# ykevinc/pocket-tts

Measured on AMD Instinct MI355X. Metric: audio-sec/wall-sec (RTF) per GPU at batch=32 + p50 first-chunk latency, higher is better.
Workload: dtype f32; 1 GPU; b6369a24 batch=32 concurrent 10 s utterances per GPU (125 frames, voice prompt 125 frames, 40 text tokens), lsd_decode_steps=1 (BASELINE configs[2]); global_batch=32, utterance_frames=125, jobs=37, prompt_frames=125, parallelism=replicas x1

## Files before the change

pocket-tts_amd/csrc/capi.cpp:

```cpp
#include <cstdlib>
#include <cstring>
#include <string>

#include "engine.h"
#include "flac_join.h"
#include "pocket_tts.h"
#include "pocket_tts_probe.h"
#include "test_hooks.h"

struct ptts_engine {
  ptts::Engine* impl = nullptr;
};

namespace {
thread_local std::string g_err;

template <class F>
int guard(F&& f) {
  try {
    f();
    g_err.clear();
    return PTTS_OK;
  } catch (const ptts::Error& e) {
    g_err = e.what();
// ... 158 lines not shown
}

int ptts_resample(ptts_engine* e, const float* x, int n_samples, int sr_from, int sr_to, float* y) {
  return guard([&] { eng(e).resample_host(x, n_samples, sr_from, sr_to, y); });
}

int ptts_resample_len_ex(int n_samples, int sr_from, int sr_to, int resampler) {
  if (resampler == PTTS_RESAMPLE_POLY) return ptts_resample_len(n_samples, sr_from, sr_to);
  if (resampler != PTTS_RESAMPLE_RUBATO_SEPTIC || n_samples <= 0 || sr_from <= 0 || sr_to <= 0) return 0;
  if (sr_from == sr_to) return n_samples;
  const long n = ptts::septic_schedule(n_samples, sr_from, sr_to, nullptr, nullptr);
  return n < (1L << 30) ? (int)n : 0;
}

int ptts_resample_ex(ptts_engine* e, const float* x, int n_samples, int sr_from, int sr_to, int resampler, float* y) {
  return guard([&] { eng(e).resample_host(x, n_samples, sr_from, sr_to, y, resampler); });
}

int ptts_voice_from_audio_ex(ptts_engine* e, const float* samples, int n_samples, int sample_rate, int chunk_frames,
                             int resampler, ptts_voice** out) {
  return guard([&] {
    if (!out) throw ptts::Error(PTTS_ERR_INVALID, "null out");
    *out = eng(e).voice_from_audio(samples, n_samples, sample_rate, chunk_frames, resampler);
  });
}

int ptts_test_gemm(ptts_engine* e, int layout, int m, int n, int k, int splits, int tail_slices, const float* x,
                   const float* w, float* y) {
  return guard([&] { eng(e).test_gemm(layout, m, n, k, splits, tail_slices, x, w, y); });
}

int ptts_test_attention(ptts_engine* e, int kind, int m, int nh, int cap, int window, int n_slots, int splits,
                        const float* qkv, float* kv, const float* pre, const int* pre_len, int slot0, int rps, int p0,
                        const int* pos, const int* tab, const int* ptab, int mpad, float* q, float* o) {
  return guard([&] {
    eng(e).test_attention(kind, m, nh, cap, window, n_slots, splits, qkv, kv, pre, pre_len, slot0, rps, p0, pos, tab,
                          ptab, mpad, q, o);
  });
}

int ptts_test_align(ptts_engine* e, int m, int nh, int cap, int splits, const float* qkv, const float* kv,
                    const float* pre, const int* pre_len, const int* pos, const int* tab, unsigned head_mask,
                    float* out) {
  return guard([&] { eng(e).test_align(m, nh, cap, splits, qkv, kv, pre, pre_len, pos, tab, head_mask, out); });
}

int ptts_test_row_reduce(ptts_engine* e, int m, int n, int splits, int act, int ln, float eps, int front,
                         const float* p, const float* bias, const float* gate, const float* r, const float* ln_w,
                         const float* ln_b, const float* mscale, const float* mshift, float* y, float* h,
                         float* hfrag) {
  return guard([&] {
    eng(e).test_row_reduce(m, n, splits, act, ln, eps, front, p, bias, gate, r, ln_w, ln_b, mscale, mshift, y, h, hfrag);
  });
}

int ptts_voice_job_start(ptts_engine* e, const void* samples, int n_samples, int sample_format, int sample_rate,
                         int chunk_frames, int resampler, ptts_voice** out) {
  return guard([&] {
    if (!out) throw ptts::Error(PTTS_ERR_INVALID, "null out");
    *out = nullptr;
    *out = eng(e).voice_job_audio(samples, n_samples, sample_format, sample_rate, chunk_frames, resampler);
  });
}

int ptts_voice_job_start_prompt(ptts_engine* e, const float* prompt, int n_frames, ptts_voice** out) {
  return guard([&] {
    if (!out) throw ptts::Error(PTTS_ERR_INVALID, "null out");
    *out = nullptr;
    *out = eng(e).voice_job_prompt(prompt, n_frames);
  });
}

int ptts_voice_ready(const ptts_voice* v, int wait, int* ready) {
  return guard([&] {
    if (!ready) throw ptts::Error(PTTS_ERR_INVALID, "null argument");
    *ready = 1;
    if (!v || !v->ev) return;
    if (wait) {
      PTTS_HIP(hipEventSynchronize(v->ev));
      return;
    }
    const hipError_t q = hipEventQuery(v->ev);
    if (q == hipErrorNotReady) *ready = 0;
    else PTTS_HIP(q);
  });
}

int ptts_voice_jobs_reserve(ptts_engine* e, int max_frames) {
  return guard([&] { eng(e).voice_jobs_reserve(max_frames); });
}

int ptts_voice_len(const ptts_voice* v) { return v ? v->F : 0; }

int ptts_voice_conditioning(const ptts_voice* v, float* out, int max_rows) {
  return guard([&] {
    if (!v || !out) throw ptts::Error(PTTS_ERR_INVALID, "null argument");
    if (v->cond.empty() && !v->h_cond) throw ptts::Error(PTTS_ERR_STATE, "voice was not built from PCM");
    const int rows = std::min(max_rows, v->F);
    if (v->h_cond) {
      PTTS_HIP(hipEventSynchronize(v->ev));
      memcpy(out, v->h_cond, sizeof(float) * rows * ptts::D);
      return;
    }
    memcpy(out, v->cond.data(), sizeof(float) * rows * ptts::D);
  });
}
// ... 311 lines not shown
```

pocket-tts_amd/csrc/engine.cpp:

```cpp
#include "engine.h"

#include <hip/hip_ext.h>

#include <algorithm>
#include <array>
#include <cstdlib>
#include <cmath>
#include <cstring>
#include <mutex>

namespace ptts {

namespace {
std::mutex& voice_mu() {
  static std::mutex m;
  return m;
}

int pick_splits(int M, int N, int K) {
  const int tiles = ((N + 31) / 32) * ((M + 31) / 32);
  const int chunks = K / 32;
  int s = std::max(1, 768 / std::max(1, tiles));
  s = std::min(s, std::max(1, chunks / 4));
  return std::min(s, 16);
// ... 557 lines not shown
      use.push_back(&q);
      bytes += ((size_t)q.N * q.K + 255) / 256 * 256;
    }
  }
  if (use.empty()) return;
  void* codes = nullptr;
  PTTS_HIP(hipMalloc(&codes, bytes));
  allocs_.push_back(codes);
  int* bad = (int*)dalloc(1);
  size_t off = 0;
  for (const Layout::Q8* q : use) {
    int8_t* c = (int8_t*)codes + off;
    quant_codes(W(q->w), W(q->s), q->N, q->K, c, bad, stream_);
    q8map_[W(q->w)] = {c, W(q->s)};
    off += ((size_t)q->N * q->K + 255) / 256 * 256;
  }
  PTTS_HIP(hipGetLastError());
  int nbad = 0;
  PTTS_HIP(hipMemcpyAsync(&nbad, bad, sizeof(int), hipMemcpyDeviceToHost, stream_));
  PTTS_HIP(hipStreamSynchronize(stream_));
  if (nbad) {
    q8map_.clear();
    throw Error(PTTS_ERR_INVALID, "quantized weights are not on their int8 grid (" + std::to_string(nbad) +
                                      " elements): blob not packed by the quantizer");
  }
}

void Engine::derive_fp8() {
  std::vector<const Layout::Q8*> use;
  size_t bytes = 0, nsc = 0;
  for (const Layout::Q8& q : L_.q8)
    if ((long)q.N * q.K >= (2L << 20)) {
      use.push_back(&q);
      bytes += ((size_t)q.N * q.K + 255) / 256 * 256;
      nsc += (size_t)q.N;
    }
  void* codes = nullptr;
  PTTS_HIP(hipMalloc(&codes, std::max<size_t>(bytes, 1)));
  allocs_.push_back(codes);
  float* scales = dalloc(nsc);
  size_t off = 0, so = 0;
  for (const Layout::Q8* q : use) {
    uint8_t* c = (uint8_t*)codes + off;
    fp8_codes(W(q->w), q->N, q->K, c, scales + so, stream_);
    f8map_[W(q->w)] = {c, scales + so};
    off += ((size_t)q->N * q->K + 255) / 256 * 256;
    so += (size_t)q->N;
  }
  PTTS_HIP(hipGetLastError());
  PTTS_HIP(hipStreamSynchronize(stream_));
}

void Engine::linear_split(std::vector<Op>& ops, const std::string& name, const float* X, long ldx, int M,
                          const float* Wt, int N, int K, int* S_out, const FlowBufs& fb) {
  PTTS_REQUIRE(K % 32 == 0, "GEMM K must be a multiple of 32");
  int S = pick_splits(M, N, K);
  int layout = TILE_KSPLIT_4W, tail = 0;
  if (M <= 64 && N >= 3072) {
    layout = TILE_GLDS_32x128;
    S = std::max(1, std::min(8, K / 64));
  } else if (M >= 256) {
    layout = N >= 4096 && K <= 1024 ? TILE_ILV_128x64 : TILE_ILV_128x64_2CU;
    tail = N >= 4096 && K <= 1024 ? 2 : 4;
    S = 1;
  } else if (M <= 64 && K >= 4096) {
    S = 8;
  } else if (M <= 64 && N <= 512 && K == 512) {
    layout = TILE_KSPLIT_8W;
    S = 8;
  }
  auto gv = gvmap_.find(Wt);
  if (gv != gvmap_.end() && M <= 64 && (gemv_mask_ & gv->second.bit)) {
    const GemvShape g = gv->second.g;
    const float* P = gv->second.packed;
    const uint32_t* q8 = gv->second.q8;
    const float* sc = gv->second.scale;
    const int Sg = K / g.ks();
    PTTS_REQUIRE((size_t)Sg * M * N <= fb.pcap, "split-K partial buffer too small");
    float* part = fb.partial;
    const bool f8 = fp8_ && q8;
    ops.push_back({name, [=](hipStream_t s) { gemv_splitk(X, ldx, M, N, K, P, g, part, s, q8, sc, f8); }, 2.0 * M * N * K,
                   (q8 ? 1.0 * N * K + 4.0 * N : 4.0 * N * K) + 4.0 * ((double)M * K + (double)Sg * M * N)});
    *S_out = Sg;
    return;
  }
  auto f8 = f8map_.find(Wt);
  const bool wf8 = f8 != f8map_.end() && M <= 64;
  if (wf8) {
    layout = TILE_KSPLIT_4W;
    const int tiles = ((N + 63) / 64) * ((M + 31) / 32), nch = K / 32;
    S = 1;
    while (S < 16 && tiles * S < 256 && nch / (2 * S) >= 4) S *= 2;
    while ((nch + S - 1) / S > FP8_KSLICE_MAX / 32) ++S;
  }
  auto q8 = q8map_.find(Wt);
  const bool w8 = q8 != q8map_.end() && M <= 64 && (long)N * K >= (2L << 20);
  if (w8) {
    layout = TILE_KSPLIT_4W;
    const int tiles = ((N + 63) / 64) * ((M + 31) / 32);
    S = 1;
    while (S < 16 && tiles * S < 256 && (K / 32) / (2 * S) >= 4) S *= 2;
  }
  if (!w8 && !wf8) tile_override(name, layout, S);
  while (S > 1 && (size_t)S * M * N > fb.pcap) --S;
  PTTS_REQUIRE((size_t)S * M * N <= fb.pcap, "split-K partial buffer too small");
  GemmArgs a = dense_gemm(layout, M, N, K, X, ldx, Wt);
  if (w8) {
    a.Wq = q8->second.first;
    a.wscale = q8->second.second;
  }
  if (wf8) {
    PTTS_REQUIRE((K / 32 + S - 1) / S <= FP8_KSLICE_MAX / 32, "fp8 GEMM K slice too long");
    a.Wf8 = f8->second.first;
    a.wscale = f8->second.second;
  }
  a.S = S;
  a.partial = fb.partial;
  if (tail > 0 && S == 1 && !w8 && !wf8) {
    a.tail_S = tail;
    a.tail_slab = fb.tslab;
    a.tail_cap = fb.tail_cap;
    a.tickets = fb.tickets;
    a.tickets_cap = TICKETS;
  }
  a.w_nt = M <= 64 && layout != TILE_KSPLIT_4W;
  a.front = 1;
  ops.push_back({name, [a, S](hipStream_t s) { gemm(a, S, s); }, 2.0 * M * N * K,
                 (w8 || wf8 ? (double)N * K + 4.0 * N : 4.0 * N * K) + 4.0 * ((double)M * K + (double)S * M * N)});
  *S_out = S;
}

static Op rr_op(const std::string& name, const RowReduceArgs& a) {
  const double mn = (double)a.M * a.N;
  double f = mn * (a.S + 1 + (a.act ? 8 : 0) + (a.ln ? 8 : 0));
  double b = mn * a.S + (a.bias ? a.N : 0) + (a.gate ? (a.ldg ? mn : a.N) : 0) + (a.R ? mn : 0) + (a.Y ? mn : 0) +
             (a.Y2 ? mn : 0) + (a.euler ? 2.0 * a.M * 32 : 0);
  if (a.ln) b += mn + (a.ln_w ? 2.0 * a.N : 0) + (a.mshift ? 2.0 * mn : 0);
  if (a.fhm) b += mn * 2.0 / 3.0;
  if (a.fill) b += 4.0 * a.fill_n4;
  if (a.x0_hx) {
    b += (double)a.x0_B * (32 + 512) + 32.0 * 512;
    f += 2.0 * a.x0_B * 32 * 512;
  }
  return Op{name, [a](hipStream_t s) { row_reduce(a, s); }, f, 4.0 * b};
}

void Engine::push_rr(std::vector<Op>& ops, const std::string& name, const RowReduceArgs& r) {
  RowReduceArgs a = r;
  a.front = 1;
  ops.push_back(rr_op(name, a));
}

void Engine::dense_op(std::vector<Op>& ops, const std::string& name, const float* X, int M, const float* Wt, int N,
                      int K, const float* bias, int act, const float* rscale, const float* R, float* Y, int layout) {
  int ks = 1;
  tile_override(name, layout, ks);
  PTTS_REQUIRE(K % tile_of(layout).bk == 0, "GEMM K must be a multiple of the tile's BK");
  GemmArgs a = dense_gemm(layout, M, N, K, X, K, Wt);
  a.S = 1;
  a.bias = bias;
  a.act = act;
  a.rscale = rscale;
  a.R = R;
  a.ldr = N;
  a.Y = Y;
  a.ldy = N;
  attach_split(a);
  ops.push_back({name, [a](hipStream_t s) { gemm(a, 1, s); }, 2.0 * M * N * K,
                 4.0 * ((double)N * K + (double)M * K + (double)M * N * (R ? 2 : 1))});
}

void Engine::conv_op(std::vector<Op>& ops, const std::string& name, const float* X, int B, int T_in, int cin,
                     const float* H, int P, int stride, int elu, const float* Wt, int cout, int ktaps, int phases,
                     const float* bias, const float* R, float* Y, int T_out, int tstride, int layout, int elu_out,
                     float* Y2, int ksplit, float* slabs, size_t slab_cap) {
  tile_override(name, layout, ksplit);
  const TileInfo& tile = tile_of(layout);
  PTTS_REQUIRE(cin % tile.bk == 0, "conv cin must be a multiple of the tile's BK");
  PTTS_REQUIRE(ksplit == 1 || (phases == 1 && tile.lds_dma()), "K-split convs need a single-phase LDS-DMA tile");
  GemmArgs a{};
  a.mode = 1;
  a.layout = layout;
  a.Tq = T_in / stride;
  a.M = B * a.Tq;
  a.N = cout;
  a.K = ktaps * cin;
  a.Nw = (cout + 31) / 32 * 32;
  a.X = X;
  a.ldx = cin;
  a.H = H;
  a.P = P;
  a.T_in = T_in;
  a.stride_in = stride;
  a.cin = cin;
  a.elu_in = elu;
  a.W = Wt;
  a.w_phase_stride = (long)cout * ktaps * cin;
  a.S = 1;
  a.bias = bias;
  a.R = R;
  a.ldr = cout;
  a.Y = Y;
  a.ldy = cout;
  a.T_out = T_out;
  a.out_tstride = tstride;
  a.elu_out = elu_out;
  a.Y2 = Y2;
  const int nph = phases;
  attach_split(a);
  if (ksplit > 1) {
    PTTS_REQUIRE((size_t)ksplit * a.M * a.N <= slab_cap, "back split-K slab buffer too small");
    a.S = ksplit;
    a.partial = slabs;
    phases = ksplit;
  }
  ops.push_back({name, [a, phases](hipStream_t s) { gemm(a, phases, s); }, 2.0 * a.M * a.N * a.K * nph,
                 4.0 * ((double)nph * a.N * a.K + (double)B * T_in * cin +
                        (double)B * T_out * cout * ((R ? 2 : 1) + (Y2 ? 1 : 0)))});
}

void Engine::flow_layers(std::vector<Op>& ops, int M, RowMap map, bool step, bool out_norm, const std::string& tag,
                         const FlowBufs& fb, float* align_out) {
  PTTS_REQUIRE(!step || &fb == &fbm_, "step passes run on the engine's own buffers");
  for (int l = 0; l < NL; ++l) {
    const Layout::TL& t = L_.fl[l];
    const std::string p = tag + ".l" + std::to_string(l);
    KvStore kv = fb.kv;
    kv.base += (long)l * fb.kv_layer;
    if (kv.pre) kv.layer = l;
    int S = 1;
    linear_split(ops, p + ".qkv_gemm", fb.h, D, M, W(t.in_proj), 3 * D, D, &S, fb);
    if (step) {
      const float* P = fb.partial;
      float* O = fb.o;
      const float* rope = rope_;
      const double L = plan_ctx_ > 0 ? plan_ctx_ : max_ctx_ / 2.0;
      const double kvu = plan_kvu_ > 0 ? plan_kvu_ : M * L;
      ops.push_back({p + ".attention", [=](hipStream_t s) { attention_step_qkv(P, S, M, NH, map, kv, rope, O, s); },
                     (double)M * 4096.0 * L,
                     8192.0 * kvu + (double)M * (4.0 * (S * 3.0 * D + 2.0 * D + D) + 64.0 * 4 * 2)});
      if (align_out && l == align_layer_) {
        AlignArgs a{};
        a.P = P;
        a.S = S;
        a.M = M;
        a.nh = NH;
        a.pos = map.pos_arr;
        a.kv = kv;
        a.rope = rope;
        a.tab = align_tab_;
        a.head_mask = align_mask_;
        a.out = align_out;
        double rows = 0, keys = 0;
        for (int b = 0; b < M; ++b)
          if (slot_align_[b]) rows += 1, keys += slot_align_[b];
        const double h = __builtin_popcount(align_mask_);
        ops.push_back({p + ".align", [=](hipStream_t s) { align_step(a, s); }, h * keys * (128.0 + 8.0),
                       h * (256.0 * keys + rows * 4.0 * (S * 64.0 + 64.0)) + rows * 4.0 * ALIGN_ROW +
                           (M - rows) * 4.0 + M * 12.0});
      }
    } else {
      {
        const float* P = fb.partial;
        float* Q = fb.q;
        ops.push_back({p + ".qkv_rope", [=](hipStream_t s) { qkv_rope_append(P, S, nullptr, M, NH, map, kv, Q, s); }});
      }
      const float* Q = fb.q;
      float* O = fb.o;
      RowMap am = map;
      int Ma = M;
      if (map.ptab) {
        am.tab = map.ptab;
        Ma = map.mpad;
      }
      ops.push_back({p + ".attention", [=](hipStream_t s) { attention(Q, Ma, NH, am, kv, 0, O, s); }});
    }
    auto rr = [&](const std::string& name, int S2, int N, int act, bool resid, float* Y, const float* lnw,
                  const float* lnb, bool ln, float* Hout, float* Hfrag = nullptr, float* fill = nullptr,
                  long fill_n4 = 0) {
      RowReduceArgs a{};
      a.Hfrag = Hfrag;
      a.fill = fill;
      a.fill_n4 = fill_n4;
// ... 2 lines not shown
      a.M = M;
      a.N = N;
      a.act = act;
      if (resid) {
        a.R = fb.x;
        a.ldr = D;
      }
      a.Y = Y;
      a.ldy = N;
      a.ln = ln ? 1 : 0;
      a.ln_w = lnw;
      a.ln_b = lnb;
      a.eps = 1e-5f;
      a.Hout = Hout;
      a.ldh = N;
      push_rr(ops, name, a);
    };
    linear_split(ops, p + ".out_gemm", fb.o, D, M, W(t.out_proj), D, D, &S, fb);
    auto fk = step && gemv_fk_supported(M, FF, D) ? fkmap_.find(W(t.l1)) : fkmap_.end();
    const bool use_fk = fk != fkmap_.end() && hfrag_;
    rr(p + ".out_reduce_ln2", S, D, ACT_NONE, true, fb.x, W(t.n2w), W(t.n2b), true, fb.h, use_fk ? hfrag_ : nullptr);
    auto ffn = use_fk && ffn_hand_ ? ffnmap_.find(W(t.l2)) : ffnmap_.end();
    if (ffn != ffnmap_.end()) {
      static_assert(NL % 2 == 0, "the fused FFN's hand-off sets alternate by layer");
      const float *A = hfrag_, *P1 = fk->second, *P2 = ffn->second;
      float *hand = ffn_hand_, *Pp = fb.partial;
      int* err = herr_;
      const int set = l & 1;
      const int groups = ffn_groups_;
      auto f8 = ffn8map_.find(W(t.l2));
      const uint32_t *Q1 = nullptr, *Q2 = nullptr;
      const float *s1 = nullptr, *s2 = nullptr;
      if (f8 != ffn8map_.end()) {
        Q1 = f8->second.first.first;
        s1 = f8->second.first.second;
        Q2 = f8->second.second.first;
        s2 = f8->second.second.second;
      }
      const bool e4m3 = fp8_ && Q1;
      Op op{p + ".ffn", [=](hipStream_t s) { ffn_fused(A, M, P1, P2, groups, hand, set, Pp, err, s, Q1, s1, Q2, s2, e4m3); },
            2.0 * M * FF * D * 2,
            (Q1 ? 2.0 * FF * D + 8.0 * (FF + D) : 8.0 * FF * D) + 4.0 * ((double)M * D + (double)groups * M * D)};
      op.prep = [hand](hipStream_t s) { PTTS_HIP(hipMemsetD32Async(hand, 0xFFFFFFFFu, 2 * FFN_HAND_FLOATS, s)); };
      ops.push_back(op);
      S = groups;
    } else {
      if (use_fk) {
        const float* Pk = fk->second;
        const float* A = hfrag_;
        float* U = fb.u;
        ops.push_back({p + ".ff1_gemm", [=](hipStream_t s) { gemv_fk(A, M, FF, Pk, nullptr, ACT_GELU, U, FF, s); },
                       2.0 * M * FF * D, 4.0 * ((double)FF * D + (double)M * D + (double)M * FF)});
      } else {
        linear_split(ops, p + ".ff1_gemm", fb.h, D, M, W(t.l1), FF, D, &S, fb);
        rr(p + ".ff1_reduce_gelu", S, FF, ACT_GELU, false, fb.u, nullptr, nullptr, false, nullptr);
      }
      linear_split(ops, p + ".ff2_gemm", fb.u, FF, M, W(t.l2), D, FF, &S, fb);
    }
    if (l + 1 < NL)
      rr(p + ".ff2_reduce_ln1", S, D, ACT_NONE, true, fb.x, W(L_.fl[l + 1].n1w), W(L_.fl[l + 1].n1b), true, fb.h);
    else {
      const bool pre = step && out_norm && use_head_prelude(M);
      const long n4 = (long)lsd_ * ((M + 15) / 16) * HP_REGION_FLOATS / 4;
      rr(p + ".ff2_reduce_outnorm", S, D, ACT_NONE, true, fb.x, W(L_.out_norm_w), W(L_.out_norm_b), out_norm, fb.h,
         pre ? hfrag_ : nullptr, pre ? hp_hand_ : nullptr, pre ? n4 : 0);
    }
  }
}

void Engine::prefill_rows(std::vector<Op>& ops, int slot, int T, int p0, const FlowBufs& fb) {
  {
    float *x = fb.x, *h = fb.h;
    const float* w = W(L_.fl[0].n1w);
    const float* b = W(L_.fl[0].n1b);
    ops.push_back({"prefill.ln1", [=](hipStream_t s) { layernorm(x, D, h, D, T, D, w, b, 1e-5f, s); }});
  }
  RowMap map{slot, T, p0, nullptr};
  flow_layers(ops, T, map, false, false, "prefill", fb);
}

bool Engine::use_head_chain(int B) const {
  if (!flow_head_fits(B)) return false;
  if (flow_head_grid(B) > head_resident_) return false;
  return head_uniform_stride();
}

bool Engine::use_head_prelude(int B) const {
  return hp_w_ && head_prelude_supported(B, 1) && gemv_fk_supported(B, NCOND_PAD, D) && use_head_chain(B);
}

bool Engine::head_uniform_stride() const {
  const long s = (long)(L_.rb_w0[1] - L_.rb_w0[0]);
  for (int i = 1; i < FDEPTH; ++i)
    if ((long)(L_.rb_lnw[i] - L_.rb_lnw[i - 1]) != s || (long)(L_.rb_lnb[i] - L_.rb_lnb[i - 1]) != s ||
        (long)(L_.rb_w0[i] - L_.rb_w0[i - 1]) != s || (long)(L_.rb_b0[i] - L_.rb_b0[i - 1]) != s ||
        (long)(L_.rb_w2[i] - L_.rb_w2[i - 1]) != s || (long)(L_.rb_b2[i] - L_.rb_b2[i - 1]) != s)
      return false;
  return true;
}

void Engine::build_front(std::vector<Op>& ops, int B, int hb, int lsd_run) {
  PTTS_REQUIRE(lsd_run >= 1 && lsd_run <= lsd_, "lsd_run outside [1, cap]");
  int S = 1;
  const FlowBufs& fb = fbm_;
  flow_layers(ops, B, RowMap{0, 1, 0, fpos_}, true, true, "flow", fb, align_ ? align_block(hb) : nullptr);
  if (use_head_prelude(B)) {
    const int RG = (B + 15) / 16;
    const size_t r0 = (size_t)(RG * 16) * FD;
// ... 1116 lines not shown
      void* p = dalloc(bytes);
      PTTS_HIP(hipMemcpyAsync(p, src, bytes, hipMemcpyHostToDevice, stream_));
      return p;
    };
    const float* dqkv = (const float*)up(qkv, sizeof(float) * n_qkv);
    float* dkv = (float*)up(kvh, sizeof(float) * n_kv);
    float* dq = (float*)dalloc(sizeof(float) * Mq * d);
    float* dout = (float*)dalloc(sizeof(float) * M * d);
    PTTS_HIP(hipMemsetAsync(dq, 0, sizeof(float) * Mq * d, stream_));
    PTTS_HIP(hipMemsetAsync(dout, 0, sizeof(float) * M * d, stream_));
    RowMap map{slot0, rps, p0, nullptr};
    if (tab) {
      map = RowMap{0, 1, 0, nullptr, (const int*)up(tab, sizeof(int) * M)};
      if (ptab) {
        map.ptab = (const int*)up(ptab, sizeof(int) * mpad);
        map.mpad = mpad;
        map.qrow = (const int*)up(qrow.data(), sizeof(int) * M);
        map.orow = (const int*)up(orow.data(), sizeof(int) * mpad);
      }
    } else if (pos) {
      map.pos_arr = (const int*)up(pos, sizeof(int) * n_slots);
    }
    KvStore kv{dkv, (long)2 * nh * cap * 64, cap};
    if (pre) {
      const float* dpre = (const float*)up(pre, sizeof(float) * pre_floats);
      for (int sl = 0; sl < n_slots; ++sl) prep[sl] = dpre + pre_off[sl];
      kv.pre = (const float* const*)up(prep.data(), sizeof(float*) * n_slots);
      kv.pre_len = (const int*)up(pre_len, sizeof(int) * n_slots);
      kv.layer = 0;
    }
    if (kind == 0) {
      qkv_rope_append(S > 0 ? dqkv : nullptr, S, S > 0 ? nullptr : dqkv, M, nh, map, kv, dq, stream_);
      RowMap am = map;
      if (map.ptab) am.tab = map.ptab;
      attention(dq, Mq, nh, am, kv, window, dout, stream_);
    } else if (kind == 1) {
      attention16_qkv(dqkv, M, nh, map, kv, window, dout, stream_);
    } else {
      float* drope = (float*)dalloc(sizeof(float) * cap * 64);
      rope_table(drope, cap, stream_);
      attention_step_qkv(dqkv, S, M, nh, map, kv, drope, dout, stream_);
    }
    PTTS_HIP(hipGetLastError());
    PTTS_HIP(hipMemcpyAsync(kvh, dkv, sizeof(float) * n_kv, hipMemcpyDeviceToHost, stream_));
    if (kind == 0) PTTS_HIP(hipMemcpyAsync(Qh, dq, sizeof(float) * Mq * d, hipMemcpyDeviceToHost, stream_));
    PTTS_HIP(hipMemcpyAsync(Oh, dout, sizeof(float) * M * d, hipMemcpyDeviceToHost, stream_));
    PTTS_HIP(hipStreamSynchronize(stream_));
  } catch (...) {
    (void)hipStreamSynchronize(stream_);
    release();
    throw;
  }
  release();
}

void Engine::test_row_reduce(int M, int N, int S, int act, int ln, float eps, int front, const float* P,
                             const float* bias, const float* gate, const float* R, const float* ln_w,
                             const float* ln_b, const float* mscale, const float* mshift, float* Y, float* H,
                             float* Hfrag) {
  PTTS_REQUIRE(ready_, "engine weights not finalized");
  PTTS_REQUIRE(P && Y && M >= 1 && M <= 4096 && N >= 4 && N <= 8192 && N % 4 == 0 && S >= 1 && S <= 16,
               "test_row_reduce: bad shape");
  PTTS_REQUIRE(act == ACT_NONE || act == ACT_GELU, "test_row_reduce: act is none or GELU");
  PTTS_REQUIRE(!ln || (N <= 1024 && H), "test_row_reduce: LayerNorm rows are at most 1024 wide");
  PTTS_REQUIRE((ln_w == nullptr) == (ln_b == nullptr) && (mscale == nullptr) == (mshift == nullptr),
               "test_row_reduce: ln_w with ln_b, mscale with mshift");
  PTTS_REQUIRE(ln || (!ln_w && !mshift && !Hfrag), "test_row_reduce: affine, modulate and hfrag need ln");
  PTTS_REQUIRE(!Hfrag || (N == FK_K && M <= 32), "test_row_reduce: hfrag needs n == 1024 and m <= 32");
  sync();
  std::vector<void*> allocs;
  auto release = [&]() {
    for (void* p : allocs) (void)hipFree(p);
  };
  try {
    auto dalloc = [&](size_t floats) {
      void* p = nullptr;
      PTTS_HIP(hipMalloc(&p, sizeof(float) * std::max<size_t>(floats, 4)));
      allocs.push_back(p);
      return (float*)p;
    };
    auto up = [&](const float* src, size_t floats) -> float* {
      if (!src) return nullptr;
      float* p = dalloc(floats);
      PTTS_HIP(hipMemcpyAsync(p, src, sizeof(float) * floats, hipMemcpyHostToDevice, stream_));
      return p;
    };
    const size_t mn = (size_t)M * N;
    RowReduceArgs a{};
    a.P = up(P, (size_t)S * mn);
    a.S = S, a.M = M, a.N = N;
    a.bias = up(bias, N);
    a.act = act;
    a.gate = up(gate, mn), a.ldg = N;
    a.R = up(R, mn), a.ldr = N;
    a.Y = dalloc(mn), a.ldy = N;
    a.ln = ln ? 1 : 0;
    a.ln_w = up(ln_w, N), a.ln_b = up(ln_b, N);
    a.eps = eps;
    a.mscale = up(mscale, mn), a.mshift = up(mshift, mn), a.ldm = N;
    a.front = front ? 1 : 0;
    if (ln) a.Hout = dalloc(mn), a.ldh = N;
    if (Hfrag) {
      a.Hfrag = dalloc(FK_A_FLOATS);
      PTTS_HIP(hipMemsetAsync(a.Hfrag, 0, sizeof(float) * FK_A_FLOATS, stream_));
    }
    row_reduce(a, stream_);
// ... 1807 lines not shown
```

pocket-tts_amd/csrc/engine.h:

```cpp
#pragma once
#include <functional>
#include <map>
#include <string>
#include <vector>

#include "common.h"
#include "kernels.h"
#include "weights.h"

struct ptts_voice {
  int F = 0;
  float* kv = nullptr;
  std::vector<float> cond;
  const void* owner = nullptr;
  mutable int refs = 0;
  mutable bool dead = false;
  hipEvent_t ev = nullptr;
  float* h_cond = nullptr;
  mutable bool ordered = false;
};

namespace ptts {

struct VoicePlan;
// ... 36 lines not shown
  void slots_open(int n, const int* slots, const ptts_voice* const* voices, const int32_t* ids, const int* n_ids,
                  const ptts_gen_params* params, const ptts_slot_opts* opts);
  int lsd_cap() const { return lsd_; }
  int lsd_last_run() const { return lsd_last_run_; }
  void slot_close(int slot);
  void slots_cancel(int n, const int* slots);
  void set_latent(int slot, const float* lat);
  void decode_latents(int slot, const float* lat, int n, float* pcm, float* quant, float* up, float* tr);

  void step_async(int B);
  void flush_async(int B);
  void sync();
  void fetch(int B, float* pcm, uint8_t* valid, uint8_t* last, float* eos, float* lat, int calls_back = 0);
  bool fetch_ready(int calls_back);
  bool front_done(int calls_back, bool wait);

  void preview_enable(int max_rows);
  int preview_fetch(int wait, int max_n, int* slots, float* pcm);

  void wire_enable(bool on);
  bool wire() const { return wire_; }
  void fetch_wire(int calls_back, int B, unsigned char* out, size_t row_stride, int* n_bytes);
  static long wire_len(long n_samples, int rate, int enc);
  void wire_encode_host(const float* pcm, int n, int rate, int enc, unsigned char* out);
  void tempo_enable(bool on);
  bool tempo() const { return tempo_; }
  int wire_chunk_max() const { return level_ ? WIRE_CHUNK_MAX_LEVEL : tempo_ ? WIRE_CHUNK_MAX_TEMPO : WIRE_CHUNK_MAX; }
  void tempo_host(const float* pcm, int n, int sp, float* out);
  void pitch_enable(bool on);
  bool pitch() const { return pitch_; }
  void pitch_host(const float* x, int n, unsigned step, float* y);
  void level_enable(bool on, int ceiling_cdb);
  bool level() const { return level_; }
  long level_min_chunk() const;
  void level_host(const float* x, int n, int gain_cdb, int ceiling_cdb, float* y);
  void flac_enable(bool on);
  bool flac() const { return flac_; }
  static long flac_bound(long n);
  void flac_encode_host(const int16_t* x, int n, int rate, long long first, unsigned char* out, int* n_bytes,
                        int* index, int* n_frames);
  void fetch_flac_index(int calls_back, int B, int* index, int* n_frames);

  void align_enable(bool on, int layer, unsigned head_mask);
  bool align() const { return align_; }
  void fetch_align(int calls_back, int B, float* out, size_t row_stride, int* n_tokens);
  void test_align(int M, int nh, int cap, int S, const float* qkv, const float* kvh, const float* pre,
                  const int* pre_len, const int* pos, const int* tab, unsigned head_mask, float* out);

  double time_op(int B, const std::string& name, int reps);
  void test_gemm(int layout, int M, int N, int K, int splits, int tail_S, const float* X, const float* Wt, float* Y);
  void test_attention(int kind, int M, int nh, int cap, int window, int n_slots, int S, const float* qkv, float* kvh,
                      const float* pre, const int* pre_len, int slot0, int rps, int p0, const int* pos, const int* tab,
                      const int* ptab, int mpad, float* Qh, float* Oh);
  void test_row_reduce(int M, int N, int S, int act, int ln, float eps, int front, const float* P, const float* bias,
                       const float* gate, const float* R, const float* ln_w, const float* ln_b, const float* mscale,
                       const float* mshift, float* Y, float* H, float* Hfrag);
  void overlap_probe(int B, int reps, double* us);
  std::vector<std::string> plan_names(int B);
  int int8_matrices() const { return (int)q8map_.size(); }
  int fp8_matrices() const { return (int)f8map_.size(); }

 private:
  float* dalloc(size_t n);
  void* halloc(size_t bytes);
  const float* W(size_t off) const { return blob_ + off; }
  void upload_weights(TensorSource* src);
  void derive_int8();
  void derive_fp8();
  struct FlowBufs {
    float *x = nullptr, *h = nullptr, *q = nullptr, *o = nullptr, *u = nullptr, *partial = nullptr;
    size_t pcap = 0;
    float* tslab = nullptr;
    long tail_cap = 0;
    int* tickets = nullptr;
    KvStore kv{};
    long kv_layer = 0;
  };
  FlowBufs fbm_{};
  struct BackBufs {
    float *ring = nullptr, *qprev = nullptr, *qcur = nullptr, *mx = nullptr, *mh = nullptr, *mq = nullptr,
          *mo = nullptr, *mqkv = nullptr, *mu = nullptr, *a0 = nullptr, *mpartial = nullptr, *fin_side = nullptr;
    float *cb[3] = {}, *cv[3] = {}, *ca[3] = {}, *ce[3] = {}, *hist[8] = {};
    int* mpos = nullptr;
    size_t mpcap = 0;
  };
  BackBufs bbm_{};
  BackBufs back_alloc(int rows, int nfr);
  struct BackPass {
    int nfr = 1;
    const float* lat[NFR_MAX] = {};
    const FrameFlags* flags[NFR_MAX] = {};
    float* pcm = nullptr;
    long pcm_ld = FRAME;
    unsigned char* wire = nullptr;
    bool commit = true;
  };
  BackPass step_pass(int hb, int nfr) const;
  ResetArgs reset_args(int n) const;
  void prefill_rows(std::vector<Op>& ops, int slot, int T, int p0, const FlowBufs& fb);
  void run_ops(const std::vector<Op>& ops);
  void run_ops_on(const std::vector<Op>& ops, hipStream_t s);
  std::vector<Op> build_step(int B);
  void build_front(std::vector<Op>& ops, int B, int hb, int lsd_run);
  void build_back(std::vector<Op>& ops, int B, const BackBufs& bb, const BackPass& pass);
  hipGraphExec_t part_graph(int part, int B, int hb, int qp, int nfr, int lsd_run = 0);
  void wait_unless_done(hipStream_t s, hipEvent_t e);
  void copy_out(int B, int hb, hipStream_t s);
  void push_rr(std::vector<Op>& ops, const std::string& name, const RowReduceArgs& r);
  void flow_layers(std::vector<Op>& ops, int M, RowMap map, bool step, bool out_norm, const std::string& tag,
                   const FlowBufs& fb, float* align_out = nullptr);
  void linear_split(std::vector<Op>& ops, const std::string& name, const float* X, long ldx, int M, const float* Wt,
                    int N, int K, int* S_out, const FlowBufs& fb);
  void conv_op(std::vector<Op>& ops, const std::string& name, const float* X, int B, int T_in, int cin, const float* H,
               int P, int stride, int elu, const float* Wt, int cout, int ktaps, int phases, const float* bias,
               const float* R, float* Y, int T_out, int tstride, int layout = TILE_KSPLIT_4W, int elu_out = 0,
               float* Y2 = nullptr, int ksplit = 1, float* slabs = nullptr, size_t slab_cap = 0);
  void dense_op(std::vector<Op>& ops, const std::string& name, const float* X, int M, const float* Wt, int N, int K,
                const float* bias, int act, const float* rscale, const float* R, float* Y,
                int layout = TILE_KSPLIT_4W);
  void encoder_transformer(std::vector<Op>& ops, float* x, int T, float* h, float* qkv, float* q, float* o, float* u,
                           float* ring);

  static constexpr int LSD_MAX = 64;
  int dev_ = 0, max_slots_ = 0, max_ctx_ = 0, lsd_ = 1;
  std::vector<int> slot_lsd_;
  int lsd_last_run_ = 0;
  int lsd_run_for(int B) const;
  int wq_ = 0;
  std::map<const float*, std::pair<const int8_t*, const float*>> q8map_;
  int fp8_ = 0;
  std::map<const float*, std::pair<const uint8_t*, const float*>> f8map_;
  struct Gemv {
    const float* packed;
    GemvShape g;
    int bit;
    const uint32_t* q8;
    const float* scale;
  };
  const uint32_t* pack_codes(const float* W, int N, int K, int nj, const std::function<void(const float*, float*)>& pack);
  std::map<const float*, std::pair<std::pair<const uint32_t*, const float*>, std::pair<const uint32_t*, const float*>>>
      ffn8map_;
  std::map<const float*, Gemv> gvmap_;
  std::map<const float*, const float*> fkmap_;
  float* hfrag_ = nullptr;
  std::map<const float*, const float*> ffnmap_;
  float* ffn_hand_ = nullptr;
  int ffn_groups_ = 8;
  int gemv_mask_ = 0;
  void derive_gemv();
  bool own_blob_ = true, ready_ = false;
  hipStream_t stream_ = nullptr;
  Layout L_{};
  float* blob_ = nullptr;
  std::vector<void*> allocs_, hallocs_;

  long ring_slot_ = 0, ring_layer_ = 0;
  int* fpos_ = nullptr;
  bool share_voice_ = true;
  const float** vpre_ = nullptr;
  int* vlen_ = nullptr;
  const float** h_vpre_ = nullptr;
  int* h_vlen_ = nullptr;
  std::vector<const ptts_voice*> slot_voice_;
  void voice_release(int slot, bool drained);
  SlotState* st_ = nullptr;
// ... 215 lines not shown
```

pocket-tts_amd/csrc/kernels.h:

```cpp
#pragma once
#include <hip/hip_runtime.h>

#include <cstdint>
#include <vector>

namespace ptts {

enum Act : int { ACT_NONE = 0, ACT_GELU = 1, ACT_SILU = 2, ACT_ELU = 3 };

struct SlotState;
struct RowReduceArgs {
  const float* P;
  int S, M, N;
  const float* bias;
  int act;
  const float* gate;
  long ldg;
  const float* R;
  long ldr;
  float* Y;
  long ldy;
  float* Y2;
  float* euler;
  const SlotState* euler_st;
// ... 187 lines not shown

struct GemvShape {
  int wn, kw;
  int ks() const { return kw * (4 / wn); }
};
bool gemv_supported(GemvShape g, int N, int K);
constexpr int FK_K = 1024;
constexpr long FK_A_FLOATS = 32L * FK_K;
bool gemv_fk_supported(int M, int N, int K);
void pack_gemv_fk(const float* W, int N, int K, float* packed, hipStream_t s);
void gemv_fk(const float* Afrag, int M, int N, const float* packed, const float* bias, int act, float* Y, long ldy,
             hipStream_t s);
constexpr long FFN_HAND_FLOATS = 16L * 32 * 256;
bool ffn_fused_supported(int M, int D, int FF);
void pack_ffn2(const float* W2, int groups, float* packed, hipStream_t s);
void ffn_fused(const float* Afrag, int M, const float* P1, const float* P2, int groups, float* hand, int set, float* P,
               int* err, hipStream_t s, const uint32_t* Q1 = nullptr, const float* s1 = nullptr,
               const uint32_t* Q2 = nullptr, const float* s2 = nullptr, bool fp8 = false);
void pack_gemv(const float* W, int N, int K, GemvShape g, float* packed, hipStream_t s);
void gemv_splitk(const float* X, long ldx, int M, int N, int K, const float* packed, GemvShape g, float* partial,
                 hipStream_t s, const uint32_t* q8 = nullptr, const float* scale = nullptr, bool fp8 = false);
void codes_to_f32(const int8_t* q, long n, float* out, hipStream_t s);
void codes_u8_to_f32(const uint8_t* q, long n, float* out, hipStream_t s);
void pack_q8(const float* packed_codes, long n4, int nj, uint32_t* q8, hipStream_t s);

void quant_codes(const float* W, const float* s, int N, int K, int8_t* q, int* bad, hipStream_t st);
void fp8_codes(const float* W, int N, int K, uint8_t* q, float* s, hipStream_t st);
constexpr int FP8_KSLICE_MAX = 512;

void row_reduce(const RowReduceArgs& a, hipStream_t s);

void layernorm(const float* x, long ldx, float* y, long ldy, int M, int N, const float* w, const float* b,
               float eps, hipStream_t s);

struct RowMap {
  int slot0, rps, p0;
  const int* pos_arr;
  const int* tab;
  const int* ptab = nullptr;
  int mpad = 0;
  const int* qrow = nullptr;
  const int* orow = nullptr;
};
struct KvStore {
  float* base;
  long slot_stride;
  int cap;
  const float* const* pre = nullptr;
  const int* pre_len = nullptr;
  int layer = 0;
};
void qkv_rope_append(const float* P, int S, const float* dense, int M, int nh, RowMap map, KvStore kv,
                     float* Q, hipStream_t s);

void attention16_qkv(const float* qkv, int M, int nh, RowMap map, KvStore kv, int window, float* O, hipStream_t s);
void attention(const float* Q, int M, int nh, RowMap map, KvStore kv, int window, float* O, hipStream_t s);
void attention_step_qkv(const float* P, int S, int M, int nh, RowMap map, KvStore kv, const float* rope, float* O,
                        hipStream_t s);
void rope_table(float* tab, int npos, hipStream_t s);

constexpr int ALIGN_TOKENS = 128;
constexpr int ALIGN_ROW = 1 + ALIGN_TOKENS;
struct AlignEntry {
  int t0, n;
};
struct AlignArgs {
  const float* P;
  int S, M, nh;
  const int* pos;
  KvStore kv;
  const float* rope;
  const AlignEntry* tab;
  unsigned head_mask;
  float* out;
};
void align_step(const AlignArgs& a, hipStream_t s);

struct SlotState {
  int active;
  int step;
  int eos_step;
  int frames_after_eos, max_frames;
  float temp, eos_threshold, noise_clamp;
  unsigned long long seed;
  int lsd;
};
struct FrameFlags {
  int valid;
  int last;
};

constexpr int FLOW_COND_MAX_SLABS = 16;
constexpr int temb_row0(int n) { return n * (n - 1) / 2; }
void flow_cond(const float* P, int S, int B, const float* bias, const float* temb, int lsd_run, int lsd_cap,
               const SlotState* st, float* ysilu, float* cur, float* eos_out, hipStream_t s);

constexpr int FH_D = 512, FH_L = 32, FH_DEPTH = 6;
struct FlowHeadArgs {
  int B, lsd;
  const SlotState* st;
  float* cur;
  const float* mods;
  long ldm;
  const float *in_w, *in_b;
  const float *lnw, *lnb, *w0, *b0, *w2, *b2;
  long blk;
// ... 348 lines not shown
```

pocket-tts_amd/csrc/kernels.hip:

```cpp
#include "kernels.h"

#include <cmath>
#include <stdexcept>

#include "devfn.h"

namespace ptts {

#ifdef PTTS_PROBES
#define PTTS_PROBE(a) ((a).probe)
#else
#define PTTS_PROBE(a) 0
#endif

static thread_local int g_wg_cap = 0;
void set_wg_cap(int cap) { g_wg_cap = cap; }
static thread_local int g_back_hi = 1;
void set_back_hi(int on) { g_back_hi = on; }
#ifdef PTTS_PROBES
__device__ int g_front_prio = 0;
void set_front_prio(int prio) {
  if (hipMemcpyToSymbol(HIP_SYMBOL(g_front_prio), &prio, sizeof prio) != hipSuccess)
    throw std::runtime_error("set_front_prio failed");
}
// ... 2001 lines not shown
  for (int i = 0; i < 16; ++i) {
    const int n = lane + 64 * i;
    if (n < N) y[(long)row * ldy + n] = (v[i] - mean) / den * w[n] + b[n];
  }
}
void layernorm(const float* x, long ldx, float* y, long ldy, int M, int N, const float* w, const float* b,
               float eps, hipStream_t s) {
  hipLaunchKernelGGL(k_layernorm, dim3((M + 3) / 4), dim3(256), cap_lds(k_layernorm, g_wg_cap), s, x, ldx, y, ldy, M, N, w, b, eps);
}


__global__ __launch_bounds__(256) void k_qkv_rope(const float* P, int S, const float* dense, int M, int nh,
                                                  RowMap mp, KvStore kv, float* Q) {
  const int idx = blockIdx.x * 256 + threadIdx.x;
  const int per_row = nh * 32;
  if (idx >= M * per_row) return;
  const int row = idx / per_row;
  const int rem = idx - row * per_row;
  const int hh = rem >> 5, i = rem & 31;
  const int d = nh * 64, ld = 3 * d;
  const int c = hh * 64 + 2 * i;
  float q0, q1, k0, k1, v0, v1;
  if (dense) {
    const float* pr = dense + (long)row * ld;
    q0 = pr[c]; q1 = pr[c + 1]; k0 = pr[d + c]; k1 = pr[d + c + 1]; v0 = pr[2 * d + c]; v1 = pr[2 * d + c + 1];
  } else {
    q0 = q1 = k0 = k1 = v0 = v1 = 0.f;
    for (int z = 0; z < S; ++z) {
      const float* pr = P + ((long)z * M + row) * ld;
      q0 += pr[c]; q1 += pr[c + 1]; k0 += pr[d + c]; k1 += pr[d + c + 1]; v0 += pr[2 * d + c]; v1 += pr[2 * d + c + 1];
    }
  }
  int slot, pos;
  row_slot_pos(mp, row, slot, pos);
  const float freq = expf((float)i * (-logf(10000.0f) * 2.0f / 64.0f));
  const float ang = (float)pos * freq;
  const float cs = cosf(ang), sn = sinf(ang);
  const long qr = mp.qrow ? mp.qrow[row] : row;
  Q[qr * d + c] = q0 * cs - q1 * sn;
  Q[qr * d + c + 1] = q0 * sn + q1 * cs;
  if (slot < 0) return;
  float* kb = kv.base + (long)slot * kv.slot_stride + ((long)hh * kv.cap + (pos % kv.cap)) * 64 + 2 * i;
  float* vb = kv.base + (long)slot * kv.slot_stride + ((long)(nh + hh) * kv.cap + (pos % kv.cap)) * 64 + 2 * i;
  kb[0] = k0 * cs - k1 * sn;
  kb[1] = k0 * sn + k1 * cs;
  vb[0] = v0;
  vb[1] = v1;
}

void qkv_rope_append(const float* P, int S, const float* dense, int M, int nh, RowMap map, KvStore kv, float* Q,
                     hipStream_t s) {
  const int total = M * nh * 32;
  hipLaunchKernelGGL(k_qkv_rope, dim3((total + 255) / 256), dim3(256), cap_lds(k_qkv_rope, g_wg_cap), s, P, S, dense, M, nh, map, kv, Q);
}

typedef float floatx4 __attribute__((ext_vector_type(4)));
constexpr int A16_WAVES = 8;

__device__ __forceinline__ void rope_cs(int pos, int i, float& cs, float& sn) {
  const float freq = expf((float)i * (-logf(10000.0f) * 2.0f / 64.0f));
  const float ang = (float)pos * freq;
  cs = cosf(ang);
  sn = sinf(ang);
}

template <bool RING, bool FUSE = false>
__global__ __launch_bounds__(64 * A16_WAVES) void k_attn16(const float* __restrict__ Q, int M, int nh, RowMap mp,
                                                          KvStore kv, int window, float* __restrict__ O) {
  __shared__ float s_m[A16_WAVES][16], s_l[A16_WAVES][16];
  __shared__ float s_o[A16_WAVES][16][65];
  const int lane = threadIdx.x & 63;
  const int wave = __builtin_amdgcn_readfirstlane(threadIdx.x >> 6);
  const int c = lane & 15, G = lane >> 4;
  const int row0 = blockIdx.x * 16, head = blockIdx.y;
  int nrows = min(16, M - row0);
  if (mp.tab) {
    int n = 0;
    for (int i = 0; i < nrows; ++i) n += mp.tab[row0 + i] >= 0;
    nrows = n;
  }
  if (nrows <= 0) return;
  int slot, qpos0;
  row_slot_pos(mp, row0, slot, qpos0);
  const int kmax = qpos0 + nrows - 1;
  const int kmin = window > 0 ? max(0, qpos0 - window + 1) : 0;
  const int d = nh * 64;
  const KvHead kh = kv_head(kv, slot, nh, head);
  const float* kbase = kh.kb;
  const float* vbase = kh.vb;
  const int cmask = kv.cap - 1;
  auto kidx = [&](int kp) { return RING ? (kp & cmask) : kp; };
  auto kaddr = [&](int kp) { return (FUSE || kp >= kh.F ? kbase + (long)kidx(kp) * 64 : kh.pk + (long)kp * 64); };
  auto vaddr = [&](int kp) { return (FUSE || kp >= kh.F ? vbase + (long)kidx(kp) * 64 : kh.pv + (long)kp * 64); };
  const int ntiles = (kmax - kmin + 16) / 16;
  float4 kf[4], vf[4];
  auto load = [&](int t) {
    const int kt = kmin + 16 * t;
    const float4* kr = reinterpret_cast<const float4*>(kaddr(min(kt + c, kmax)) + 16 * G);
#pragma unroll
    for (int i = 0; i < 4; ++i) kf[i] = kr[i];
#pragma unroll
    for (int sidx = 0; sidx < 4; ++sidx)
      vf[sidx] = *reinterpret_cast<const float4*>(vaddr(min(kt + 4 * G + sidx, kmax)) + 4 * c);
  };
  const bool early = FUSE && wave < ntiles && kmin + 16 * wave + 15 < qpos0;
  if (early) load(wave);
// ... 2780 lines not shown
```

pocket-tts_amd/pocket_tts_amd/engine.py:

```python

from __future__ import annotations

import ctypes as C
from dataclasses import dataclass

import numpy as np

from ._lib import (BACK_BF16, BACK_F32, BACK_F32X6, DIM, F32P, FRAME, I32P, LDIM, SAMPLES_F32, SAMPLES_S16, U8P,
                   WIRE_ALAW, WIRE_FLAC, WIRE_CHUNK_MAX, WIRE_CHUNK_MAX_LEVEL, WIRE_CHUNK_MAX_TEMPO, WIRE_NONE, WIRE_RATES, WIRE_S16, WIRE_ULAW, EngineConfig, GenParams,
                   SAMPLE_RATE, SlotOpts5, ALIGN_TOKENS, check, fptr, lib, u8ptr)
from .audio import ENCODINGS, level_cdb, pitch_cents, pitch_plan, speed_permille

WIRE_ENCODINGS = {"pcm_s16le": WIRE_S16, "ulaw": WIRE_ULAW, "alaw": WIRE_ALAW, "flac": WIRE_FLAC}


def wire_encoding_code(encoding) -> int:
    if encoding is None:
        return WIRE_NONE
    if isinstance(encoding, str):
        if encoding not in WIRE_ENCODINGS:
            raise ValueError(f"encoding must be one of {sorted(WIRE_ENCODINGS)}, got {encoding!r}")
        return WIRE_ENCODINGS[encoding]
    return int(encoding)

# ... 275 lines not shown
        return o, kv_out, q

    def test_align(self, qkv: np.ndarray, kv: np.ndarray, pos, tab, head_mask: int, out: np.ndarray, pre=None):
        qkv = np.ascontiguousarray(qkv, np.float32)
        kv = np.ascontiguousarray(kv, np.float32)
        m, two, nh, cap, hd = kv.shape
        splits = qkv.shape[0] if qkv.ndim == 3 else 0
        if two != 2 or hd != 64 or qkv.shape[-1] != 3 * nh * 64 or qkv.shape[-2] != m:
            raise ValueError("test_align: qkv / kv shapes disagree")
        pos = np.ascontiguousarray(pos, np.int32).reshape(m)
        tab = np.ascontiguousarray(tab, np.int32).reshape(m, 2)
        o = np.array(out, np.float32, order="C").reshape(m, 1 + ALIGN_TOKENS)
        pre_cat = pre_len = None
        if pre is not None:
            parts = [np.zeros((2, nh, 0, 64), np.float32) if p is None else np.ascontiguousarray(p, np.float32)
                     for p in pre]
            pre_len = np.array([p.shape[2] for p in parts], np.int32)
            pre_cat = np.concatenate([p.ravel() for p in parts] + [np.zeros(4, np.float32)])
        i32 = C.POINTER(C.c_int32)
        fn = lib().ptts_test_align
        fn.restype = C.c_int
        fn.argtypes = [C.c_void_p] + [C.c_int] * 4 + [F32P] * 3 + [i32] * 3 + [C.c_uint, F32P]
        check(fn(self.handle, m, nh, cap, splits, fptr(qkv), fptr(kv), fptr(pre_cat),
                                    None if pre_len is None else pre_len.ctypes.data_as(i32), pos.ctypes.data_as(i32),
                                    tab.ctypes.data_as(i32), int(head_mask) & 0xFFFFFFFF, fptr(o)))
        return o[:, 0].copy().view(np.int32), o[:, 1:].copy()

    def test_row_reduce(self, p: np.ndarray, *, bias=None, gate=None, r=None, act: int = 0, ln: bool = False,
                        eps: float = 1e-5, ln_w=None, ln_b=None, mscale=None, mshift=None, hfrag: bool = False,
                        front: bool = False):
        p = np.ascontiguousarray(p, np.float32)
        s, m, n = p.shape

        def arr(a, shape):
            if a is None:
                return None
            a = np.ascontiguousarray(a, np.float32)
            if a.shape != shape:
                raise ValueError(f"test_row_reduce: expected shape {shape}, got {a.shape}")
            return a

        bias, ln_w, ln_b = arr(bias, (n,)), arr(ln_w, (n,)), arr(ln_b, (n,))
        gate, r, mscale, mshift = (arr(a, (m, n)) for a in (gate, r, mscale, mshift))
        y = np.empty((m, n), np.float32)
        h = np.empty((m, n), np.float32) if ln else None
        hf = np.empty(32 * 1024, np.float32) if hfrag else None
        fn = lib().ptts_test_row_reduce
        fn.restype = C.c_int
        fn.argtypes = [C.c_void_p] + [C.c_int] * 5 + [C.c_float, C.c_int] + [F32P] * 11
        check(fn(self.handle, m, n, s, act, int(ln), eps, int(front), fptr(p), fptr(bias), fptr(gate), fptr(r),
                 fptr(ln_w), fptr(ln_b), fptr(mscale), fptr(mshift), fptr(y), fptr(h), fptr(hf)))
        return y, h, hf

    def lsd_steps(self) -> tuple[int, int]:
        cap, run = C.c_int(0), C.c_int(0)
        check(lib().ptts_lsd_steps(self.handle, C.byref(cap), C.byref(run)))
        return int(cap.value), int(run.value)

    def _row_lsd(self, params: GenerationParams) -> int:
        return int(self.lsd_decode_steps if params.lsd_steps is None else params.lsd_steps)

    def frame_lag(self) -> tuple[int, int]:
        d = C.c_int(0)
        lag = int(lib().ptts_frame_lag(self.handle, C.byref(d)))
        return lag, int(d.value)

    @staticmethod
    def check_config(cfg_yaml: str) -> None:
        check(lib().ptts_config_check(cfg_yaml.encode()))

    @staticmethod
    def gemm_tiles() -> list[dict]:
        buf = C.create_string_buffer(1 << 14)
        check(lib().ptts_gemm_tiles(buf, len(buf)))
        out = []
        for line in buf.value.decode().splitlines():
            i, tm, tn, bk, ops, tail = line.split("\t")
            out.append({"id": int(i), "tm": int(tm), "tn": int(tn), "bk": int(bk), "operands": ops, "tail": tail == "1"})
        return out

    @staticmethod
    def weight_blob_bytes() -> int:
        return int(lib().ptts_weight_blob_bytes())

    @staticmethod
    def pack_weights(seed: int = 0x5EED, weights_path: str | None = None, weight_quant: int = 0) -> np.ndarray:
        out = np.empty(Engine.weight_blob_bytes() // 4, np.float32)
        check(lib().ptts_pack_weights_ex(seed, weights_path.encode() if weights_path else None, int(weight_quant),
                                         out.ctypes.data_as(F32P), out.nbytes))
        return out

    @staticmethod
    def weight_manifest() -> list[tuple[str, tuple[int, ...]]]:
        need = C.c_size_t(0)
        check(lib().ptts_weight_manifest(None, 0, C.byref(need)))
        buf = C.create_string_buffer(need.value)
        check(lib().ptts_weight_manifest(buf, need.value, None))
        out = []
        for line in buf.value.decode().splitlines():
            name, dims = line.split("\t")
            out.append((name, tuple(int(x) for x in dims.split(",")) if dims else ()))
        return out

    @property
    def fp8_matrices(self) -> int:
        return int(lib().ptts_engine_fp8_matrices(self.handle))
# ... 282 lines not shown
```

Before: 5458 audio-sec/wall-sec.

## Skip dead last-layer work in prefill and fuse ff1 GELU into GEMM epilogue

In the non-step (prefill) path without an output norm, the last transformer layer now computes only the K/V projection and appends roped K/V to the cache, skipping Q, attention, and FFN. Those results feed nothing downstream. The ff1 GEMM on the large-M tail path now applies GELU in its epilogue and writes straight to the output, dropping the separate row-reduce launch. A test hook that disables voice sharing is also added. The last-layer shortcut relies on the prefill outputs of that layer being unused; if they are used, the result would be wrong.

```diff
diff --git a/pocket-tts_amd/csrc/capi.cpp b/pocket-tts_amd/csrc/capi.cpp
--- a/pocket-tts_amd/csrc/capi.cpp
+++ b/pocket-tts_amd/csrc/capi.cpp
@@ -234,6 +234,10 @@
   return guard([&] {
     eng(e).test_row_reduce(m, n, splits, act, ln, eps, front, p, bias, gate, r, ln_w, ln_b, mscale, mshift, y, h, hfrag);
   });
+}
+
+int ptts_test_copy_on_admit(ptts_engine* e) {
+  return guard([&] { eng(e).test_copy_on_admit(); });
 }
 
 int ptts_voice_job_start(ptts_engine* e, const void* samples, int n_samples, int sample_format, int sample_rate,
diff --git a/pocket-tts_amd/csrc/engine.cpp b/pocket-tts_amd/csrc/engine.cpp
--- a/pocket-tts_amd/csrc/engine.cpp
+++ b/pocket-tts_amd/csrc/engine.cpp
@@ -633,20 +633,22 @@
 }
 
 void Engine::linear_split(std::vector<Op>& ops, const std::string& name, const float* X, long ldx, int M,
-                          const float* Wt, int N, int K, int* S_out, const FlowBufs& fb) {
+                          const float* Wt, int N, int K, int* S_out, const FlowBufs& fb, int act, float* Y,
+                          int N_whole) {
   PTTS_REQUIRE(K % 32 == 0, "GEMM K must be a multiple of 32");
-  int S = pick_splits(M, N, K);
+  const int Ns = N_whole > 0 ? N_whole : N;
+  int S = pick_splits(M, Ns, K);
   int layout = TILE_KSPLIT_4W, tail = 0;
-  if (M <= 64 && N >= 3072) {
+  if (M <= 64 && Ns >= 3072) {
     layout = TILE_GLDS_32x128;
     S = std::max(1, std::min(8, K / 64));
   } else if (M >= 256) {
-    layout = N >= 4096 && K <= 1024 ? TILE_ILV_128x64 : TILE_ILV_128x64_2CU;
-    tail = N >= 4096 && K <= 1024 ? 2 : 4;
+    layout = Ns >= 4096 && K <= 1024 ? TILE_ILV_128x64 : TILE_ILV_128x64_2CU;
+    tail = Ns >= 4096 && K <= 1024 ? 2 : 4;
     S = 1;
   } else if (M <= 64 && K >= 4096) {
     S = 8;
-  } else if (M <= 64 && N <= 512 && K == 512) {
+  } else if (M <= 64 && Ns <= 512 && K == 512) {
     layout = TILE_KSPLIT_8W;
     S = 8;
   }
@@ -683,7 +685,7 @@
     while (S < 16 && tiles * S < 256 && (K / 32) / (2 * S) >= 4) S *= 2;
   }
   if (!w8 && !wf8) tile_override(name, layout, S);
-  while (S > 1 && (size_t)S * M * N > fb.pcap) --S;
+  while (S > 1 && (size_t)S * M * Ns > fb.pcap) --S;
   PTTS_REQUIRE((size_t)S * M * N <= fb.pcap, "split-K partial buffer too small");
   GemmArgs a = dense_gemm(layout, M, N, K, X, ldx, Wt);
   if (w8) {
@@ -697,18 +699,27 @@
   }
   a.S = S;
   a.partial = fb.partial;
+  bool epi = false;
   if (tail > 0 && S == 1 && !w8 && !wf8) {
     a.tail_S = tail;
     a.tail_slab = fb.tslab;
     a.tail_cap = fb.tail_cap;
     a.tickets = fb.tickets;
     a.tickets_cap = TICKETS;
+    if (Y) {
+      epi = true;
+      a.partial = nullptr;
+      a.act = act;
+      a.Y = Y;
+      a.ldy = N;
+    }
   }
   a.w_nt = M <= 64 && layout != TILE_KSPLIT_4W;
   a.front = 1;
   ops.push_back({name, [a, S](hipStream_t s) { gemm(a, S, s); }, 2.0 * M * N * K,
                  (w8 || wf8 ? (double)N * K + 4.0 * N : 4.0 * N * K) + 4.0 * ((double)M * K + (double)S * M * N)});
-  *S_out = S;
+  if (epi && act != ACT_NONE) ops.back().flops += 8.0 * M * N;
+  *S_out = epi ? 0 : S;
 }
 
 static Op rr_op(const std::string& name, const RowReduceArgs& a) {
@@ -810,6 +821,24 @@
     kv.base += (long)l * fb.kv_layer;
     if (kv.pre) kv.layer = l;
     int S = 1;
+    if (!step && !out_norm && l == NL - 1) {
+      const float* Wqkv = W(t.in_proj);
+      auto gv = gvmap_.find(Wqkv);
+      const bool whole = M <= 64 && ((gv != gvmap_.end() && (gemv_mask_ & gv->second.bit)) || q8map_.count(Wqkv) ||
+                                     f8map_.count(Wqkv));
+      if (whole) {
+        linear_split(ops, p + ".qkv_gemm", fb.h, D, M, Wqkv, 3 * D, D, &S, fb);
+        const float* P = fb.partial;
+        float* Q = fb.q;
+        ops.push_back({p + ".qkv_rope", [=](hipStream_t s) { qkv_rope_append(P, S, nullptr, M, NH, map, kv, Q, s); }});
+      } else {
+        linear_split(ops, p + ".kv_gemm", fb.h, D, M, Wqkv + (size_t)D * D, 2 * D, D, &S, fb, ACT_NONE, nullptr,
+                     3 * D);
+        const float* P = fb.partial;
+        ops.push_back({p + ".kv_rope", [=](hipStream_t s) { kv_rope_append(P, S, M, NH, map, kv, s); }});
+      }
+      break;
+    }
     linear_split(ops, p + ".qkv_gemm", fb.h, D, M, W(t.in_proj), 3 * D, D, &S, fb);
     if (step) {
       const float* P = fb.partial;
@@ -918,8 +947,8 @@
         ops.push_back({p + ".ff1_gemm", [=](hipStream_t s) { gemv_fk(A, M, FF, Pk, nullptr, ACT_GELU, U, FF, s); },
                        2.0 * M * FF * D, 4.0 * ((double)FF * D + (double)M * D + (double)M * FF)});
       } else {
-        linear_split(ops, p + ".ff1_gemm", fb.h, D, M, W(t.l1), FF, D, &S, fb);
-        rr(p + ".ff1_reduce_gelu", S, FF, ACT_GELU, false, fb.u, nullptr, nullptr, false, nullptr);
+        linear_split(ops, p + ".ff1_gemm", fb.h, D, M, W(t.l1), FF, D, &S, fb, ACT_GELU, step ? nullptr : fb.u);
+        if (S > 0) rr(p + ".ff1_reduce_gelu", S, FF, ACT_GELU, false, fb.u, nullptr, nullptr, false, nullptr);
       }
       linear_split(ops, p + ".ff2_gemm", fb.u, FF, M, W(t.l2), D, FF, &S, fb);
     }
@@ -2142,6 +2171,16 @@
     throw;
   }
   release();
+}
+
+void Engine::test_copy_on_admit() {
+  PTTS_REQUIRE(ready_, "engine weights not finalized");
+  bool fresh = graphs_.empty() && pv_graphs_.empty() && k_ == 0;
+  for (const ptts_voice* v : slot_voice_) fresh = fresh && v == nullptr;
+  if (!fresh) throw Error(PTTS_ERR_STATE, "test_copy_on_admit: the engine has admitted or stepped already");
+  share_voice_ = false;
+  fbm_.kv.pre = nullptr;
+  fbm_.kv.pre_len = nullptr;
 }
 
 void Engine::test_row_reduce(int M, int N, int S, int act, int ln, float eps, int front, const float* P,
diff --git a/pocket-tts_amd/csrc/engine.h b/pocket-tts_amd/csrc/engine.h
--- a/pocket-tts_amd/csrc/engine.h
+++ b/pocket-tts_amd/csrc/engine.h
@@ -112,6 +112,7 @@
   void test_attention(int kind, int M, int nh, int cap, int window, int n_slots, int S, const float* qkv, float* kvh,
                       const float* pre, const int* pre_len, int slot0, int rps, int p0, const int* pos, const int* tab,
                       const int* ptab, int mpad, float* Qh, float* Oh);
+  void test_copy_on_admit();
   void test_row_reduce(int M, int N, int S, int act, int ln, float eps, int front, const float* P, const float* bias,
                        const float* gate, const float* R, const float* ln_w, const float* ln_b, const float* mscale,
                        const float* mshift, float* Y, float* H, float* Hfrag);
@@ -170,7 +171,8 @@
   void flow_layers(std::vector<Op>& ops, int M, RowMap map, bool step, bool out_norm, const std::string& tag,
                    const FlowBufs& fb, float* align_out = nullptr);
   void linear_split(std::vector<Op>& ops, const std::string& name, const float* X, long ldx, int M, const float* Wt,
-                    int N, int K, int* S_out, const FlowBufs& fb);
+                    int N, int K, int* S_out, const FlowBufs& fb, int act = ACT_NONE, float* Y = nullptr,
+                    int N_whole = 0);
   void conv_op(std::vector<Op>& ops, const std::string& name, const float* X, int B, int T_in, int cin, const float* H,
                int P, int stride, int elu, const float* Wt, int cout, int ktaps, int phases, const float* bias,
                const float* R, float* Y, int T_out, int tstride, int layout = TILE_KSPLIT_4W, int elu_out = 0,
diff --git a/pocket-tts_amd/csrc/kernels.h b/pocket-tts_amd/csrc/kernels.h
--- a/pocket-tts_amd/csrc/kernels.h
+++ b/pocket-tts_amd/csrc/kernels.h
@@ -263,6 +263,7 @@
 };
 void qkv_rope_append(const float* P, int S, const float* dense, int M, int nh, RowMap map, KvStore kv,
                      float* Q, hipStream_t s);
+void kv_rope_append(const float* P, int S, int M, int nh, RowMap map, KvStore kv, hipStream_t s);
 
 void attention16_qkv(const float* qkv, int M, int nh, RowMap map, KvStore kv, int window, float* O, hipStream_t s);
 void attention(const float* Q, int M, int nh, RowMap map, KvStore kv, int window, float* O, hipStream_t s);
diff --git a/pocket-tts_amd/csrc/kernels.hip b/pocket-tts_amd/csrc/kernels.hip
--- a/pocket-tts_amd/csrc/kernels.hip
+++ b/pocket-tts_amd/csrc/kernels.hip
@@ -2077,6 +2077,40 @@
                      hipStream_t s) {
   const int total = M * nh * 32;
   hipLaunchKernelGGL(k_qkv_rope, dim3((total + 255) / 256), dim3(256), cap_lds(k_qkv_rope, g_wg_cap), s, P, S, dense, M, nh, map, kv, Q);
+}
+
+__global__ __launch_bounds__(256) void k_kv_rope(const float* P, int S, int M, int nh, RowMap mp, KvStore kv) {
+  const int idx = blockIdx.x * 256 + threadIdx.x;
+  const int per_row = nh * 32;
+  if (idx >= M * per_row) return;
+  const int row = idx / per_row;
+  const int rem = idx - row * per_row;
+  const int hh = rem >> 5, i = rem & 31;
+  const int d = nh * 64, ld = 2 * d;
+  const int c = hh * 64 + 2 * i;
+  float k0, k1, v0, v1;
+  k0 = k1 = v0 = v1 = 0.f;
+  for (int z = 0; z < S; ++z) {
+    const float* pr = P + ((long)z * M + row) * ld;
+    k0 += pr[c]; k1 += pr[c + 1]; v0 += pr[d + c]; v1 += pr[d + c + 1];
+  }
+  int slot, pos;
+  row_slot_pos(mp, row, slot, pos);
+  if (slot < 0) return;
+  const float freq = expf((float)i * (-logf(10000.0f) * 2.0f / 64.0f));
+  const float ang = (float)pos * freq;
+  const float cs = cosf(ang), sn = sinf(ang);
+  float* kb = kv.base + (long)slot * kv.slot_stride + ((long)hh * kv.cap + (pos % kv.cap)) * 64 + 2 * i;
+  float* vb = kv.base + (long)slot * kv.slot_stride + ((long)(nh + hh) * kv.cap + (pos % kv.cap)) * 64 + 2 * i;
+  kb[0] = fmaf(k0, cs, -(k1 * sn));
+  kb[1] = fmaf(k1, cs, k0 * sn);
+  vb[0] = v0;
+  vb[1] = v1;
+}
+
+void kv_rope_append(const float* P, int S, int M, int nh, RowMap map, KvStore kv, hipStream_t s) {
+  const int total = M * nh * 32;
+  hipLaunchKernelGGL(k_kv_rope, dim3((total + 255) / 256), dim3(256), cap_lds(k_kv_rope, g_wg_cap), s, P, S, M, nh, map, kv);
 }
 
 typedef float floatx4 __attribute__((ext_vector_type(4)));
diff --git a/pocket-tts_amd/pocket_tts_amd/engine.py b/pocket-tts_amd/pocket_tts_amd/engine.py
--- a/pocket-tts_amd/pocket_tts_amd/engine.py
+++ b/pocket-tts_amd/pocket_tts_amd/engine.py
@@ -351,6 +351,12 @@
                  fptr(ln_w), fptr(ln_b), fptr(mscale), fptr(mshift), fptr(y), fptr(h), fptr(hf)))
         return y, h, hf
 
+    def test_copy_on_admit(self) -> None:
+        fn = lib().ptts_test_copy_on_admit
+        fn.restype = C.c_int
+        fn.argtypes = [C.c_void_p]
+        check(fn(self.handle))
+
     def lsd_steps(self) -> tuple[int, int]:
         cap, run = C.c_int(0), C.c_int(0)
         check(lib().ptts_lsd_steps(self.handle, C.byref(cap), C.byref(run)))
```

Result: no change. 5473 audio-sec/wall-sec (median of 6 runs) (+0.3%).
